# danielsuo/cuSIFT

Measured on AMD Instinct MI355X. Metric: Mpix/s pyramid + keypoints/s end-to-end, 1920x1080 batch, higher is better.
Workload: dtype f32

## Files before the change

### cusift_amd/csrc/detect_chunk.inc

```
  const int c0 = bx * kDetStrip - kDetHaloLanes * kBlurCols + lane * kBlurCols;
  const EdgeFix4 edge(c0, w);
  const __amdgpu_buffer_rsrc_t rin =
      __builtin_amdgcn_make_buffer_rsrc((void *)img, 0, (int)((unsigned int)h * (unsigned int)pitch * 4u), kBufFlags);
  const bool lane_valid = lane >= kDetHaloLanes && lane < 64 - kDetHaloLanes;

  auto load_raw = [&](int y) -> f4 {
    const int yc = clampi(__builtin_amdgcn_readfirstlane(y), 0, h - 1);
    return __builtin_bit_cast(f4, __builtin_amdgcn_raw_buffer_load_b128(rin, edge.voff, yc * pitch * 4, 0));
  };
  const bool edge_wave = bx == 0 || bx * kDetStrip - kDetHaloLanes * kBlurCols + 64 * kBlurCols > w;
  auto fix = [&](f4 v) -> f4 { return edge_wave ? edge(v) : v; };

  f4 win[9];
#pragma unroll
  for (int i = 0; i < 9; ++i) win[i] = fix(load_raw(ya - 1 - 4 + i));

  f4 DA[kNumDog], DB[kNumDog], DC[kNumDog];
#pragma unroll
  for (int p = 0; p < kNumDog; ++p) DA[p] = DB[p] = DC[p] = f4{0.f, 0.f, 0.f, 0.f};

  f2 hm1 = f2{0.f, 0.f}, h0 = hm1, hp1 = hm1;
  int voff_down = kOobOffset;
  if (kDown) {
    const bool odd0 = ((ya - 1) & 1) != 0;
    hm1 = down_hrow(odd0 ? win[4] : win[3], DT.k[0], DT.k[1], DT.k[2]);
    h0 = down_hrow(odd0 ? win[5] : win[4], DT.k[0], DT.k[1], DT.k[2]);
    hp1 = down_hrow(odd0 ? win[6] : win[5], DT.k[0], DT.k[1], DT.k[2]);
    voff_down = (lane_valid && c0 >= 0) ? (c0 >> 1) * 4 : kOobOffset;
  }

  f4 ahead = load_raw(ya - 1 + 5);
  auto row_step = [&](int yy, f4 (&D0)[kNumDog], f4 (&D1)[kNumDog], f4 (&D2)[kNumDog]) {
    const f4 nxt = ahead;
    ahead = load_raw(yy + 6);
    if (kDown) {
      const int yu = __builtin_amdgcn_readfirstlane(yy);
      if ((yu & 1) == 0) {
        const f2 hp2 = down_hrow(win[6], DT.k[0], DT.k[1], DT.k[2]), hp3 = down_hrow(win[7], DT.k[0], DT.k[1], DT.k[2]);
        const f2 o = down_vcol(hm1, h0, hp1, hp2, hp3, DT.k[0], DT.k[1], DT.k[2]);
        const int r = yu >> 1;
        if (yu >= own_lo && yu < own_hi && r < (h >> 1)) {
          const __amdgpu_buffer_rsrc_t ro = __builtin_amdgcn_make_buffer_rsrc(
              (void *)(down_img + (long)r * down_pitch), 0, (w >> 1) * 4, kBufFlags);
          __builtin_amdgcn_raw_buffer_store_b64(__builtin_bit_cast(u2, o), ro, voff_down, 0, 0);
        }
        hm1 = hp1;
        h0 = hp2;
        hp1 = hp3;
      }
    }
    blur_dog_row<kIdent0>(win, T, D2);

    if (yy >= ya + 1) {
      const int y = yy - 1;
      float vmax = 0.0f;
#pragma unroll
      for (int s = 0; s < kNumScales; ++s) {
        const f4 v = D1[s + 1];
        vmax = max3f(vmax, fabsf(v.x), fabsf(v.y));
        vmax = max3f(vmax, fabsf(v.z), fabsf(v.w));
      }
      const bool big = vmax > P.thr_pos && lane_valid && c0 < w;
      unsigned int cand = 0;
      if (__builtin_amdgcn_ballot_w64(big) != 0) {
        f4 hmn[kNumDog], hmx[kNumDog];
        f4 lmn[kNumScales], rmn[kNumScales], lmx[kNumScales], rmx[kNumScales];
#pragma unroll
        for (int p = 0; p < kNumDog; ++p) {
          f4 cmn, cmx, l_mn, r_mn, l_mx, r_mx;
#pragma unroll
          for (int j = 0; j < 4; ++j) {
            cmn[j] = min3f(D0[p][j], D1[p][j], D2[p][j]);
            cmx[j] = max3f(D0[p][j], D1[p][j], D2[p][j]);
          }
          l_mn = f4{from_prev_lane(cmn[3]), cmn[0], cmn[1], cmn[2]};
          r_mn = f4{cmn[1], cmn[2], cmn[3], from_next_lane(cmn[0])};
          l_mx = f4{from_prev_lane(cmx[3]), cmx[0], cmx[1], cmx[2]};
          r_mx = f4{cmx[1], cmx[2], cmx[3], from_next_lane(cmx[0])};
#pragma unroll
          for (int j = 0; j < 4; ++j) {
            hmn[p][j] = min3f(l_mn[j], cmn[j], r_mn[j]);
            hmx[p][j] = max3f(l_mx[j], cmx[j], r_mx[j]);
          }
          if (p >= 1 && p <= kNumScales) {
            lmn[p - 1] = l_mn;
            rmn[p - 1] = r_mn;
            lmx[p - 1] = l_mx;
            rmx[p - 1] = r_mx;
          }
        }
#pragma unroll
        for (int s = 0; s < kNumScales; ++s) {
          const int c = s + 1;
#pragma unroll
          for (int j = 0; j < 4; ++j) {
            const float v = D1[c][j];
            const float mn_a = min3f(lmn[s][j], rmn[s][j], D0[c][j]);
            const float mn_b = min3f(D2[c][j], hmn[c - 1][j], hmn[c + 1][j]);
            const float mx_a = max3f(lmx[s][j], rmx[s][j], D0[c][j]);
            const float mx_b = max3f(D2[c][j], hmx[c - 1][j], hmx[c + 1][j]);
            const bool hit = (v < min3f(mn_a, mn_b, P.thr_neg)) || (v > max3f(mx_a, mx_b, P.thr_pos));
            cand |= (hit ? 1u : 0u) << (4 * s + j);
          }
        }
      }
      if (!lane_valid) cand = 0;
#pragma unroll
      for (int j = 0; j < 4; ++j)
        if (c0 + j < 1 || c0 + j > w - 2) cand &= ~(0x11111u << j);
      if (__builtin_amdgcn_ballot_w64(cand != 0) != 0) {
#pragma unroll 1
        for (int s = 0; s < kNumScales; ++s) {
          const unsigned int m = (cand >> (4 * s)) & 0xfu;
          if (__builtin_amdgcn_ballot_w64(m != 0) == 0) continue;
          auto emit = [&](auto scale_c) {
            constexpr int k = decltype(scale_c)::value;
            auto column = [&](auto col_c) {
              constexpr int j = decltype(col_c)::value;
              const bool mine = (m >> j) & 1u;
              if (__builtin_amdgcn_ballot_w64(mine) == 0) return;
              auto at = [&](const f4 (&D)[kNumDog], int p, int dx) -> float {
                const int col = j + dx;
                if (col < 0) return from_prev_lane(D[p][3]);
                if (col > 3) return from_next_lane(D[p][0]);
                return D[p][col];
              };
              const float c00 = at(D0, k + 1, -1), c01 = at(D0, k + 1, 0), c02 = at(D0, k + 1, 1);
              const float c10 = at(D1, k + 1, -1), c11 = at(D1, k + 1, 0), c12 = at(D1, k + 1, 1);
              const float c20 = at(D2, k + 1, -1), c21 = at(D2, k + 1, 0), c22 = at(D2, k + 1, 1);
              const float l0 = at(D1, k, 0), l1 = at(D1, k, -1), l2 = at(D1, k, 1), l3 = at(D0, k, 0), l4 = at(D2, k, 0);
              const float h0 = at(D1, k + 2, 0), h1 = at(D1, k + 2, -1), h2 = at(D1, k + 2, 1), h3 = at(D0, k + 2, 0),
                          h4 = at(D2, k + 2, 0);
              float *e = cands.reserve(mine);
              if (mine) {
                e[0] = c00, e[1] = c01, e[2] = c02, e[3] = c10, e[4] = c11, e[5] = c12, e[6] = c20, e[7] = c21, e[8] = c22;
                e[9] = l0, e[10] = l1, e[11] = l2, e[12] = l3, e[13] = l4;
                e[14] = h0, e[15] = h1, e[16] = h2, e[17] = h3, e[18] = h4;
                e[19] = __builtin_bit_cast(float, c0 + j);
                e[20] = __builtin_bit_cast(float, ((y + rw.row0) << 3) | k);
              }
              if (cands.n >= 64) {
                cands.refine_batch<kRecBytes>(list, max_pts, counter, P, lane);
              }
            };
            column(std::integral_constant<int, 0>{});
            column(std::integral_constant<int, 1>{});
            column(std::integral_constant<int, 2>{});
            column(std::integral_constant<int, 3>{});
          };
          switch (s) {
            case 0: emit(std::integral_constant<int, 0>{}); break;
            case 1: emit(std::integral_constant<int, 1>{}); break;
            case 2: emit(std::integral_constant<int, 2>{}); break;
            case 3: emit(std::integral_constant<int, 3>{}); break;
            default: emit(std::integral_constant<int, 4>{}); break;
          }
        }
      }
    }
#pragma unroll
    for (int i = 0; i < 8; ++i) win[i] = win[i + 1];
    win[8] = fix(nxt);
  };

  for (int yy = ya - 1; yy <= yb; yy += 3) {
    row_step(yy, DA, DB, DC);
    if (yy + 1 > yb) break;
    row_step(yy + 1, DB, DC, DA);
    if (yy + 2 > yb) break;
    row_step(yy + 2, DC, DA, DB);
  }
  cands.refine_batch<kRecBytes>(list, max_pts, counter, P, lane);
```

### cusift_amd/csrc/sift_stencils.hip

```cpp
#include <type_traits>

#include "sift_device.h"

namespace cusift {

__global__ void __launch_bounds__(256) scale_down_kernel(float *__restrict__ dst, int dst_pitch, long dst_stride,
                                                        const float *__restrict__ src, int w, int h, int src_pitch,
                                                        long src_stride, int rows_per_wave, ScaleDownTaps T) {
  const int lane = threadIdx.x & 63;
  const int wv = __builtin_amdgcn_readfirstlane(threadIdx.x >> 6);
  const int ow = w >> 1, oh = h >> 1;
  const int c = blockIdx.x * 64 + lane;
  const int r0 = (blockIdx.y * kWavesPerBlock + wv) * rows_per_wave;
  if (r0 >= oh) return;
  const int r1 = min(r0 + rows_per_wave, oh);
  src += (long)blockIdx.z * src_stride;
  dst += (long)blockIdx.z * dst_stride;
  const int x0 = clampi(2 * c - 2, 0, w - 1), x1 = clampi(2 * c - 1, 0, w - 1), x2 = clampi(2 * c, 0, w - 1),
            x3 = clampi(2 * c + 1, 0, w - 1), x4 = clampi(2 * c + 2, 0, w - 1);
  const float k0 = T.k[0], k1 = T.k[1], k2 = T.k[2];
  auto hrow = [&](int y) -> float {
    const float *s = src + (long)clampi(y, 0, h - 1) * src_pitch;
    float v = k0 * (s[x0] + s[x4]);
    v = fmaf(k1, s[x1] + s[x3], v);
    v = fmaf(k2, s[x2], v);
    return v;
  };
  float bm1 = hrow(2 * r0 - 1), b0 = hrow(2 * r0), bp1 = hrow(2 * r0 + 1);
  for (int r = r0; r < r1; ++r) {
    const float bp2 = hrow(2 * r + 2), bp3 = hrow(2 * r + 3);
    float v = k2 * b0;
    v = fmaf(k0, bp3 + bp2, v);
    v = fmaf(k1, bm1 + bp1, v);
    if (c < ow) dst[(long)r * dst_pitch + c] = v;
    bm1 = bp1;
    b0 = bp2;
    bp1 = bp3;
  }
}

__global__ void __launch_bounds__(256) laplace_multi_kernel(const float *__restrict__ img, float *__restrict__ dog,
                                                           int w, int h, int pitch, long img_stride, long dog_stride,
                                                           int rows_per_wave, int vec_ok, LaplaceTaps T) {
  const int lane = threadIdx.x & 63;
  const int wv = __builtin_amdgcn_readfirstlane(threadIdx.x >> 6);
  const int y0 = (blockIdx.y * kWavesPerBlock + wv) * rows_per_wave;
  if (y0 >= h) return;
  const int y1 = min(y0 + rows_per_wave, h);
  img += (long)blockIdx.z * img_stride;
  dog += (long)blockIdx.z * dog_stride;

  const int c0 = blockIdx.x * kBlurStrip - kBlurHaloLanes * kBlurCols + lane * kBlurCols;
  const bool interior = vec_ok && c0 >= 0 && c0 + 3 < w;
  const int cc0 = clampi(c0, 0, w - 1), cc1 = clampi(c0 + 1, 0, w - 1), cc2 = clampi(c0 + 2, 0, w - 1),
            cc3 = clampi(c0 + 3, 0, w - 1);

  float win[9][4];
  auto load_row = [&](int y, float (&o)[4]) {
    const float *r = img + (long)clampi(y, 0, h - 1) * pitch;
    if (interior) {
      const float4 v = *reinterpret_cast<const float4 *>(r + c0);
      o[0] = v.x; o[1] = v.y; o[2] = v.z; o[3] = v.w;
    } else {
      o[0] = r[cc0]; o[1] = r[cc1]; o[2] = r[cc2]; o[3] = r[cc3];
    }
  };
#pragma unroll
  for (int i = 0; i < 8; ++i) load_row(y0 - 4 + i, win[i]);

  const bool writer = lane >= kBlurHaloLanes && lane < 64 - kBlurHaloLanes && c0 < w;
  const bool vec_store = vec_ok && (c0 + 3 < w);
  const long plane = (long)h * pitch;

  for (int y = y0; y < y1; ++y) {
    load_row(y + 4, win[8]);
    float ctr[4], p1[4], p2[4], p3[4], p4[4];
#pragma unroll
    for (int j = 0; j < 4; ++j) {
      ctr[j] = win[4][j];
      p1[j] = win[3][j] + win[5][j];
      p2[j] = win[2][j] + win[6][j];
      p3[j] = win[1][j] + win[7][j];
      p4[j] = win[0][j] + win[8][j];
    }
    float prevL[4];
    float *out = dog + (long)y * pitch + c0;
#pragma unroll
    for (int s = 0; s < kNumLevels; ++s) {
      const float k0 = T.k[s][0], k1 = T.k[s][1], k2 = T.k[s][2], k3 = T.k[s][3], k4 = T.k[s][4];
      float e[12];
#pragma unroll
      for (int j = 0; j < 4; ++j) {
        float v = k4 * ctr[j];
        v = fmaf(k3, p1[j], v);
        v = fmaf(k2, p2[j], v);
        v = fmaf(k1, p3[j], v);
        v = fmaf(k0, p4[j], v);
        e[4 + j] = v;
      }
#pragma unroll
      for (int j = 0; j < 4; ++j) {
        e[j] = from_prev_lane(e[4 + j]);
        e[8 + j] = from_next_lane(e[4 + j]);
      }
      float L[4];
#pragma unroll
      for (int j = 0; j < 4; ++j) {
        const int m = 4 + j;
        float v = k4 * e[m];
        v = fmaf(k3, e[m - 1] + e[m + 1], v);
        v = fmaf(k2, e[m - 2] + e[m + 2], v);
        v = fmaf(k1, e[m - 3] + e[m + 3], v);
        v = fmaf(k0, e[m - 4] + e[m + 4], v);
        L[j] = v;
      }
      if (s > 0 && writer) {
        float *o = out + (long)(s - 1) * plane;
        if (vec_store) {
          *reinterpret_cast<float4 *>(o) =
              make_float4(prevL[0] - L[0], prevL[1] - L[1], prevL[2] - L[2], prevL[3] - L[3]);
        } else {
#pragma unroll
          for (int j = 0; j < 4; ++j)
            if (c0 + j < w) o[j] = prevL[j] - L[j];
        }
      }
#pragma unroll
      for (int j = 0; j < 4; ++j) prevL[j] = L[j];
    }
#pragma unroll
    for (int i = 0; i < 8; ++i)
#pragma unroll
      for (int j = 0; j < 4; ++j) win[i][j] = win[i + 1][j];
  }
}

__device__ __forceinline__ f2 splat(float v) { return f2{v, v}; }
__device__ __forceinline__ f2 pk_fma(f2 a, f2 b, f2 c) { return __builtin_elementwise_fma(a, b, c); }
__device__ __forceinline__ f2 dpp_prev2(f2 v) { return f2{from_prev_lane(v.x), from_prev_lane(v.y)}; }
__device__ __forceinline__ f2 dpp_next2(f2 v) { return f2{from_next_lane(v.x), from_next_lane(v.y)}; }

template <int kStoreAux>
__global__ void __launch_bounds__(256) laplace_multi_fast_kernel(const float *__restrict__ img,
                                                                float *__restrict__ dog, int w, int h, int pitch,
                                                                long img_stride, long dog_stride, int rows_per_wave,
                                                                LaplaceTapsPk T) {
  const int lane = threadIdx.x & 63;
  const int wv = __builtin_amdgcn_readfirstlane(threadIdx.x >> 6);
  int bx = blockIdx.x, by = blockIdx.y, bz = blockIdx.z;
  xcd_remap(bx, by, bz);
  const int y0 = (by * (int)(blockDim.x >> 6) + wv) * rows_per_wave;
  if (y0 >= h) return;
  const int y1 = min(y0 + rows_per_wave, h);
  img += (long)bz * img_stride;
  dog += (long)bz * dog_stride;

  const int c0 = bx * kBlurStrip - kBlurHaloLanes * kBlurCols + lane * kBlurCols;
  const EdgeFix4 edge(c0, w);
  const __amdgpu_buffer_rsrc_t rin =
      __builtin_amdgcn_make_buffer_rsrc((void *)img, 0, (int)((unsigned int)h * (unsigned int)pitch * 4u), kBufFlags);
  const int voff_out = (lane >= kBlurHaloLanes && lane < 64 - kBlurHaloLanes) ? c0 * 4 : kOobOffset;
  const long plane = (long)h * pitch;

  auto load_row = [&](int y) -> f4 {
    const int yc = clampi(y, 0, h - 1);
    const u4 raw = __builtin_amdgcn_raw_buffer_load_b128(rin, edge.voff, yc * pitch * 4, 0);
    return edge(__builtin_bit_cast(f4, raw));
  };

  f4 win[9];
#pragma unroll
  for (int i = 0; i < 9; ++i) win[i] = load_row(y0 - 4 + i);

  for (int y = y0; y < y1; ++y) {
    const f4 nxt = load_row(y + 5);
    const f4 ctr = win[4];
    const f4 p1 = win[3] + win[5];
    const f4 p2 = win[2] + win[6];
    const f4 p3 = win[1] + win[7];
    const f4 p4 = win[0] + win[8];
    float *row = dog + (long)y * pitch;
    float prev_hi[4];
#pragma unroll
    for (int q = 0; q < kNumLevels / 2; ++q) {
      const f2 k0 = T.k[q][0], k1 = T.k[q][1], k2 = T.k[q][2], k3 = T.k[q][3], k4 = T.k[q][4];
      f2 e[12];
#pragma unroll
      for (int j = 0; j < 4; ++j) {
        f2 v = k4 * splat(ctr[j]);
        v = pk_fma(k3, splat(p1[j]), v);
        v = pk_fma(k2, splat(p2[j]), v);
        v = pk_fma(k1, splat(p3[j]), v);
        v = pk_fma(k0, splat(p4[j]), v);
        e[4 + j] = v;
      }
#pragma unroll
      for (int j = 0; j < 4; ++j) {
        e[j] = dpp_prev2(e[4 + j]);
        e[8 + j] = dpp_next2(e[4 + j]);
      }
      f2 L[4];
#pragma unroll
      for (int j = 0; j < 4; ++j) {
        const int m = 4 + j;
        f2 v = k4 * e[m];
        v = pk_fma(k3, e[m - 1] + e[m + 1], v);
        v = pk_fma(k2, e[m - 2] + e[m + 2], v);
        v = pk_fma(k1, e[m - 3] + e[m + 3], v);
        v = pk_fma(k0, e[m - 4] + e[m + 4], v);
        L[j] = v;
      }
      if (q > 0) {
        const f4 d = f4{prev_hi[0] - L[0].x, prev_hi[1] - L[1].x, prev_hi[2] - L[2].x, prev_hi[3] - L[3].x};
        const __amdgpu_buffer_rsrc_t ro =
            __builtin_amdgcn_make_buffer_rsrc((void *)(row + (long)(2 * q - 1) * plane), 0, w * 4, kBufFlags);
        __builtin_amdgcn_raw_buffer_store_b128(__builtin_bit_cast(u4, d), ro, voff_out, 0, kStoreAux);
      }
      {
        const f4 d = f4{L[0].x - L[0].y, L[1].x - L[1].y, L[2].x - L[2].y, L[3].x - L[3].y};
        if (2 * q < kNumDog) {
          const __amdgpu_buffer_rsrc_t ro =
              __builtin_amdgcn_make_buffer_rsrc((void *)(row + (long)(2 * q) * plane), 0, w * 4, kBufFlags);
          __builtin_amdgcn_raw_buffer_store_b128(__builtin_bit_cast(u4, d), ro, voff_out, 0, kStoreAux);
        }
      }
#pragma unroll
      for (int j = 0; j < 4; ++j) prev_hi[j] = L[j].y;
    }
#pragma unroll
    for (int i = 0; i < 8; ++i) win[i] = win[i + 1];
    win[8] = nxt;
  }
}
template __global__ void laplace_multi_fast_kernel<2>(const float *, float *, int, int, int, long, long, int, LaplaceTapsPk);

constexpr int kDownStrip = 62 * 2;

__device__ __forceinline__ f2 down_hrow(const f4 v, float k0, float k1, float k2) {
  const float m2 = from_prev_lane(v.z), m1 = from_prev_lane(v.w), p4 = from_next_lane(v.x);
  float a = k0 * (m2 + v.z);
  a = fmaf(k1, m1 + v.y, a);
  a = fmaf(k2, v.x, a);
  float b = k0 * (v.x + p4);
  b = fmaf(k1, v.y + v.w, b);
  b = fmaf(k2, v.z, b);
  return f2{a, b};
}
__device__ __forceinline__ f2 down_vcol(f2 bm1, f2 b0, f2 bp1, f2 bp2, f2 bp3, float k0, float k1, float k2) {
  f2 v;
#pragma unroll
  for (int j = 0; j < 2; ++j) {
    float t = k2 * b0[j];
    t = fmaf(k0, bp3[j] + bp2[j], t);
    t = fmaf(k1, bm1[j] + bp1[j], t);
    v[j] = t;
  }
  return v;
}

__global__ void __launch_bounds__(256) scale_down_fast_kernel(float *__restrict__ dst, int dst_pitch, long dst_stride,
                                                             const float *__restrict__ src, int w, int h,
                                                             int src_pitch, long src_stride, int rows_per_wave,
                                                             ScaleDownTaps T, RowWindow src_rw, int dst_row0,
                                                             int r_begin, int r_end) {
  const int lane = threadIdx.x & 63;
  const int wv = __builtin_amdgcn_readfirstlane(threadIdx.x >> 6);
  int bx = blockIdx.x, by = blockIdx.y, bz = blockIdx.z;
  xcd_remap(bx, by, bz);
  const int ow = w >> 1;
  const int strip = bx * kWavesPerBlock + wv;
  const int r0 = r_begin + by * rows_per_wave;
  if (strip * kDownStrip >= ow || r0 >= r_end) return;
  const int r1 = min(r0 + rows_per_wave, r_end);
  src += (long)bz * src_stride;
  dst += (long)bz * dst_stride;

  const int cs = strip * (2 * kDownStrip) - 4 + lane * 4;
  const EdgeFix4 edge(cs, w);
  const __amdgpu_buffer_rsrc_t rin = __builtin_amdgcn_make_buffer_rsrc(
      (void *)src, 0, (int)((unsigned int)h * (unsigned int)src_pitch * 4u), kBufFlags);
  const int o0 = cs >> 1;
  const int voff_out = (lane >= 1 && lane <= 62 && cs >= 0) ? o0 * 4 : kOobOffset;
  const float k0 = T.k[0], k1 = T.k[1], k2 = T.k[2];

  auto load_row = [&](int y) -> f4 {
    const u4 raw = __builtin_amdgcn_raw_buffer_load_b128(rin, edge.voff, local_row(y, h, src_rw) * src_pitch * 4, 0);
    return edge(__builtin_bit_cast(f4, raw));
  };
  auto hrow = [&](const f4 v) -> f2 { return down_hrow(v, k0, k1, k2); };

  f2 bm1 = hrow(load_row(2 * r0 - 1)), b0 = hrow(load_row(2 * r0)), bp1 = hrow(load_row(2 * r0 + 1));
  f4 n2 = load_row(2 * r0 + 2), n3 = load_row(2 * r0 + 3);
  for (int r = r0; r < r1; ++r) {
    const f4 s2 = n2, s3 = n3;
    n2 = load_row(2 * r + 4);
    n3 = load_row(2 * r + 5);
    const f2 bp2 = hrow(s2), bp3 = hrow(s3);
    const f2 v = down_vcol(bm1, b0, bp1, bp2, bp3, k0, k1, k2);
    const __amdgpu_buffer_rsrc_t ro =
        __builtin_amdgcn_make_buffer_rsrc((void *)(dst + (long)(r - dst_row0) * dst_pitch), 0, ow * 4, kBufFlags);
    __builtin_amdgcn_raw_buffer_store_b64(__builtin_bit_cast(u2, v), ro, voff_out, 0, 0);
    bm1 = bp1;
    b0 = bp2;
    bp1 = bp3;
  }
}

struct RefinedPoint {
  float x, y, scale, sharpness, edgeness;
};

__device__ __forceinline__ bool refine_from_values(const float (&c)[9], const float (&lo)[5], const float (&hi)[5], int x,
                                                   int y, int s, const FindParams &P, RefinedPoint &r) {
  const float val = c[4];
  const float dxx = 2.0f * val - c[3] - c[5];
  const float dyy = 2.0f * val - c[1] - c[7];
  const float dxy = 0.25f * (c[8] + c[0] - c[2] - c[6]);
  const float tra = dxx + dyy;
  const float det = dxx * dyy - dxy * dxy;
  if (!(tra * tra < P.edge_limit * det)) return false;
  const float edge = (tra * tra) / det;
  const float dx = 0.5f * (c[5] - c[3]);
  const float dy = 0.5f * (c[7] - c[1]);
  const float ds = 0.5f * (lo[0] - hi[0]);
  const float dss = 2.0f * val - hi[0] - lo[0];
  const float dxs = 0.25f * (hi[2] + lo[1] - lo[2] - hi[1]);
  const float dys = 0.25f * (hi[4] + lo[3] - hi[3] - lo[4]);
  const float idxx = dyy * dss - dys * dys;
  const float idxy = dys * dxs - dxy * dss;
  const float idxs = dxy * dys - dyy * dxs;
  const float idet = 1.0f / (idxx * dxx + idxy * dxy + idxs * dxs);
  const float idyy = dxx * dss - dxs * dxs;
  const float idys = dxy * dxs - dxx * dys;
  const float idss = dxx * dyy - dxy * dxy;
  float pdx = idet * (idxx * dx + idxy * dy + idxs * ds);
  float pdy = idet * (idxy * dx + idyy * dy + idys * ds);
  float pds = idet * (idxs * dx + idys * dy + idss * ds);
  if (pdx < -0.5f || pdx > 0.5f || pdy < -0.5f || pdy > 0.5f || pds < -0.5f || pds > 0.5f) {
    pdx = dx / dxx;
    pdy = dy / dyy;
    pds = ds / dss;
  }
  const float dval = 0.5f * (dx * pdx + dy * pdy + ds * pds);
  r.x = (float)x + pdx;
  r.y = (float)y + pdy;
  r.scale = P.scales[s] * sm_exp2f(pds * P.factor);
  r.sharpness = val + dval;
  r.edgeness = edge;
  return true;
}

__device__ __forceinline__ void load_candidate(const float *__restrict__ dog, long plane, int pitch, int x, int y, int s,
                                               float (&c)[9], float (&lo)[5], float (&hi)[5]) {
  const float *d1 = dog + (long)(s + 1) * plane + (long)y * pitch + x;
  const float *d0 = d1 - plane;
  const float *d2 = d1 + plane;
#pragma unroll
  for (int r = 0; r < 3; ++r)
#pragma unroll
    for (int k = 0; k < 3; ++k) c[3 * r + k] = d1[(r - 1) * pitch + (k - 1)];
  lo[0] = d0[0], lo[1] = d0[-1], lo[2] = d0[1], lo[3] = d0[-pitch], lo[4] = d0[pitch];
  hi[0] = d2[0], hi[1] = d2[-1], hi[2] = d2[1], hi[3] = d2[-pitch], hi[4] = d2[pitch];
}

__device__ __forceinline__ bool refine_from_planes(const float *__restrict__ dog, long plane, int pitch, int x, int y,
                                                   int s, const FindParams &P, RefinedPoint &r) {
  float c[9], lo[5], hi[5];
  load_candidate(dog, plane, pitch, x, y, s, c, lo, hi);
  return refine_from_values(c, lo, hi, x, y, s, P, r);
}

constexpr int kPosCap = 128;
struct PosList {
  unsigned int *buf;
  int n;
  __device__ __forceinline__ void push(bool mine, int x, int y, int s) {
    const unsigned long long m = __builtin_amdgcn_ballot_w64(mine);
    if (m == 0) return;
    const int rank = __builtin_amdgcn_mbcnt_hi((unsigned int)(m >> 32), __builtin_amdgcn_mbcnt_lo((unsigned int)m, 0u));
    if (mine) {
      buf[2 * (n + rank)] = (unsigned int)x | ((unsigned int)s << 28);
      buf[2 * (n + rank) + 1] = (unsigned int)y;
    }
    n += __builtin_popcountll(m);
  }
  __device__ __forceinline__ void refine_batch(const float *__restrict__ dog, long plane, int pitch,
                                               cusift_point *__restrict__ pts, int max_pts, unsigned int *counter,
                                               const FindParams &P, int lane) {
    const int cnt = n < 64 ? n : 64;
    if (cnt == 0) return;
    n -= cnt;
    asm volatile("s_waitcnt lgkmcnt(0)" ::: "memory");
    RefinedPoint r;
    bool accept = false;
    if (lane < cnt) {
      const unsigned int xs = buf[2 * (n + lane)], y = buf[2 * (n + lane) + 1];
      accept = refine_from_planes(dog, plane, pitch, (int)(xs & 0x0fffffffu), (int)y, (int)(xs >> 28), P, r);
    }
    const unsigned long long m = __builtin_amdgcn_ballot_w64(accept);
    if (m == 0) return;
    const int rank = __builtin_amdgcn_mbcnt_hi((unsigned int)(m >> 32), __builtin_amdgcn_mbcnt_lo((unsigned int)m, 0u));
    unsigned int base = 0;
    if (lane == 0) base = atomicAdd(counter, (unsigned int)__builtin_popcountll(m));
    base = __builtin_amdgcn_readfirstlane(base);
    const unsigned int idx = base + (unsigned int)rank;
    if (accept && idx < (unsigned int)max_pts) {
      cusift_point *pt = pts + idx;
      pt->coords2D[0] = r.x;
      pt->coords2D[1] = r.y;
      pt->scale = r.scale;
      pt->sharpness = r.sharpness;
      pt->edgeness = r.edgeness;
      pt->subsampling = P.subsampling;
    }
  }
};

__device__ __forceinline__ void refine_and_append(const float *__restrict__ dog, long plane, int pitch, int x, int y,
                                                   int s, const FindParams &P, cusift_point *__restrict__ pts,
                                                   int max_pts, unsigned int *counter) {
  RefinedPoint r;
  if (!refine_from_planes(dog, plane, pitch, x, y, s, P, r)) return;
  const unsigned int idx = atomicAdd(counter, 1u);
  if (idx >= (unsigned int)max_pts) return;
  cusift_point *pt = pts + idx;
  pt->coords2D[0] = r.x;
  pt->coords2D[1] = r.y;
  pt->scale = r.scale;
  pt->sharpness = r.sharpness;
  pt->edgeness = r.edgeness;
  pt->subsampling = P.subsampling;
}

__global__ void __launch_bounds__(256) find_points_kernel(const float *__restrict__ dog, int w, int h, int pitch,
                                                         long dog_stride, cusift_point *__restrict__ points,
                                                         int max_pts, unsigned int *__restrict__ counters,
                                                         int rows_per_wave, int vec_ok, FindParams P) {
  const int lane = threadIdx.x & 63;
  const int wv = __builtin_amdgcn_readfirstlane(threadIdx.x >> 6);
  const int y0 = (blockIdx.y * kWavesPerBlock + wv) * rows_per_wave;
  if (y0 >= h) return;
  const int y1 = min(y0 + rows_per_wave, h);
  dog += (long)blockIdx.z * dog_stride;
  points += (long)blockIdx.z * max_pts;
  unsigned int *counter = counters + blockIdx.z;

  const int c0 = blockIdx.x * kFindStrip - kFindCols + lane * kFindCols;
  const bool interior = vec_ok && c0 >= 0 && c0 + 1 < w;
  const int cc0 = clampi(c0, 0, w - 1), cc1 = clampi(c0 + 1, 0, w - 1);
  const long plane = (long)h * pitch;

  float d[kNumDog][3][2];
  auto load_rows = [&](int y, int slot) {
    const float *r = dog + (long)clampi(y, 0, h - 1) * pitch;
#pragma unroll
    for (int p = 0; p < kNumDog; ++p) {
      if (interior) {
        const float2 v = *reinterpret_cast<const float2 *>(r + (long)p * plane + c0);
        d[p][slot][0] = v.x;
        d[p][slot][1] = v.y;
      } else {
        d[p][slot][0] = r[(long)p * plane + cc0];
        d[p][slot][1] = r[(long)p * plane + cc1];
      }
    }
  };
  load_rows(y0 - 1, 0);
  load_rows(y0, 1);
  const bool lane_valid = lane >= 1 && lane <= 62;

  for (int y = y0; y < y1; ++y) {
    load_rows(y + 1, 2);
    float cmin[kNumDog][2], cmax[kNumDog][2], nmin[kNumDog][2][2], nmax[kNumDog][2][2];
#pragma unroll
    for (int p = 0; p < kNumDog; ++p) {
#pragma unroll
      for (int j = 0; j < 2; ++j) {
        cmin[p][j] = fminf(fminf(d[p][0][j], d[p][1][j]), d[p][2][j]);
        cmax[p][j] = fmaxf(fmaxf(d[p][0][j], d[p][1][j]), d[p][2][j]);
      }
      nmin[p][0][0] = from_prev_lane(cmin[p][1]);
      nmin[p][0][1] = cmin[p][1];
      nmin[p][1][0] = cmin[p][0];
      nmin[p][1][1] = from_next_lane(cmin[p][0]);
      nmax[p][0][0] = from_prev_lane(cmax[p][1]);
      nmax[p][0][1] = cmax[p][1];
      nmax[p][1][0] = cmax[p][0];
      nmax[p][1][1] = from_next_lane(cmax[p][0]);
    }
    unsigned int cand = 0;
#pragma unroll
    for (int s = 0; s < kNumScales; ++s) {
      const int c = s + 1;
#pragma unroll
      for (int j = 0; j < 2; ++j) {
        const float v = d[c][1][j];
        float mn = fminf(fminf(nmin[c - 1][j][0], cmin[c - 1][j]), nmin[c - 1][j][1]);
        mn = fminf(mn, fminf(fminf(nmin[c + 1][j][0], cmin[c + 1][j]), nmin[c + 1][j][1]));
        mn = fminf(mn, fminf(fminf(nmin[c][j][0], nmin[c][j][1]), fminf(d[c][0][j], d[c][2][j])));
        float mx = fmaxf(fmaxf(nmax[c - 1][j][0], cmax[c - 1][j]), nmax[c - 1][j][1]);
        mx = fmaxf(mx, fmaxf(fmaxf(nmax[c + 1][j][0], cmax[c + 1][j]), nmax[c + 1][j][1]));
        mx = fmaxf(mx, fmaxf(fmaxf(nmax[c][j][0], nmax[c][j][1]), fmaxf(d[c][0][j], d[c][2][j])));
        const bool hit = (v < P.thr_neg && v < mn) || (v > P.thr_pos && v > mx);
        cand |= (hit ? 1u : 0u) << (2 * s + j);
      }
    }
    if (!lane_valid) cand = 0;
    if (cand) {
      for (int b = 0; b < 2 * kNumScales; ++b) {
        if (cand & (1u << b)) {
          const int x = c0 + (b & 1), s = b >> 1;
          if (x >= 1 && x <= w - 2 && y >= 1 && y <= h - 2)
            refine_and_append(dog, plane, pitch, x, y, s, P, points, max_pts, counter);
        }
      }
    }
#pragma unroll
    for (int p = 0; p < kNumDog; ++p)
#pragma unroll
      for (int j = 0; j < 2; ++j) {
        d[p][0][j] = d[p][1][j];
        d[p][1][j] = d[p][2][j];
      }
  }
}

__device__ __forceinline__ float min3f(float a, float b, float c) { return fminf(fminf(a, b), c); }
__device__ __forceinline__ float max3f(float a, float b, float c) { return fmaxf(fmaxf(a, b), c); }

__global__ void __launch_bounds__(256) find_points_fast_kernel(const float *__restrict__ dog, int w, int h, int pitch,
                                                              long dog_stride, cusift_point *__restrict__ points,
                                                              int max_pts, unsigned int *__restrict__ counters,
                                                              int rows_per_wave, FindParams P) {
  const int lane = threadIdx.x & 63;
  const int wv = __builtin_amdgcn_readfirstlane(threadIdx.x >> 6);
  int bx = blockIdx.x, by = blockIdx.y, bz = blockIdx.z;
  xcd_remap(bx, by, bz);
  const int strip = bx * kWavesPerBlock + wv;
  const int y0 = by * rows_per_wave;
  if (strip * kFindStrip >= w || y0 >= h) return;
  const int y1 = min(y0 + rows_per_wave, h);
  dog += (long)bz * dog_stride;
  points += (long)bz * max_pts;
  unsigned int *counter = counters + bz;

  const int c0 = strip * kFindStrip - kFindCols + lane * kFindCols;
  const EdgeFix2 edge(c0, w);
  const long plane = (long)h * pitch;
  const int plane_bytes = (int)((unsigned int)h * (unsigned int)pitch * 4u);
  const __amdgpu_buffer_rsrc_t rin =
      __builtin_amdgcn_make_buffer_rsrc((void *)dog, 0, (int)((unsigned int)plane_bytes * (unsigned int)kNumDog), kBufFlags);

  auto load_row = [&](int y, f2 (&o)[kNumDog]) {
    const int row_off = clampi(y, 0, h - 1) * pitch * 4;
#pragma unroll
    for (int p = 0; p < kNumDog; ++p) {
      const u2 raw = __builtin_amdgcn_raw_buffer_load_b64(rin, edge.voff, p * plane_bytes + row_off, 0);
      o[p] = edge(__builtin_bit_cast(f2, raw));
    }
  };

  __shared__ unsigned int s_cands[kWavesPerBlock][2 * kPosCap];
  PosList cands{s_cands[wv], 0};
  f2 r0[kNumDog], r1[kNumDog], r2[kNumDog], nxt[kNumDog];
  load_row(y0 - 1, r0);
  load_row(y0, r1);
  load_row(y0 + 1, r2);
  const bool lane_valid = lane >= 1 && lane <= 62;

  for (int y = y0; y < y1; ++y) {
    load_row(y + 2, nxt);
    float cmn[kNumDog][2], cmx[kNumDog][2], hmn[kNumDog][2], hmx[kNumDog][2], lmn[kNumDog], rmn[kNumDog],
        lmx[kNumDog], rmx[kNumDog];
#pragma unroll
    for (int p = 0; p < kNumDog; ++p) {
#pragma unroll
      for (int j = 0; j < 2; ++j) {
        cmn[p][j] = min3f(r0[p][j], r1[p][j], r2[p][j]);
        cmx[p][j] = max3f(r0[p][j], r1[p][j], r2[p][j]);
      }
      lmn[p] = from_prev_lane(cmn[p][1]);
      rmn[p] = from_next_lane(cmn[p][0]);
      lmx[p] = from_prev_lane(cmx[p][1]);
      rmx[p] = from_next_lane(cmx[p][0]);
      hmn[p][0] = min3f(lmn[p], cmn[p][0], cmn[p][1]);
      hmn[p][1] = min3f(cmn[p][0], cmn[p][1], rmn[p]);
      hmx[p][0] = max3f(lmx[p], cmx[p][0], cmx[p][1]);
      hmx[p][1] = max3f(cmx[p][0], cmx[p][1], rmx[p]);
    }
    unsigned int cand = 0;
#pragma unroll
    for (int s = 0; s < kNumScales; ++s) {
      const int c = s + 1;
#pragma unroll
      for (int j = 0; j < 2; ++j) {
        const float v = r1[c][j];
        const float nl_mn = j == 0 ? lmn[c] : cmn[c][0], nr_mn = j == 0 ? cmn[c][1] : rmn[c];
        const float nl_mx = j == 0 ? lmx[c] : cmx[c][0], nr_mx = j == 0 ? cmx[c][1] : rmx[c];
        const float mn_a = min3f(nl_mn, nr_mn, r0[c][j]);
        const float mn_b = min3f(r2[c][j], hmn[c - 1][j], hmn[c + 1][j]);
        const float mx_a = max3f(nl_mx, nr_mx, r0[c][j]);
        const float mx_b = max3f(r2[c][j], hmx[c - 1][j], hmx[c + 1][j]);
        const bool hit = (v < min3f(mn_a, mn_b, P.thr_neg)) || (v > max3f(mx_a, mx_b, P.thr_pos));
        cand |= (hit ? 1u : 0u) << (2 * s + j);
      }
    }
    if (!lane_valid) cand = 0;
    if (__builtin_amdgcn_ballot_w64(cand != 0) != 0) {
      for (int b = 0; b < 2 * kNumScales; ++b) {
        const int x = c0 + (b & 1), s = b >> 1;
        const bool mine = (cand & (1u << b)) && x >= 1 && x <= w - 2 && y >= 1 && y <= h - 2;
        cands.push(mine, x, y, s);
        if (cands.n >= 64) cands.refine_batch(dog, plane, pitch, points, max_pts, counter, P, lane);
      }
    }
#pragma unroll
    for (int p = 0; p < kNumDog; ++p) {
      r0[p] = r1[p];
      r1[p] = r2[p];
      r2[p] = nxt[p];
    }
  }
  cands.refine_batch(dog, plane, pitch, points, max_pts, counter, P, lane);
}

constexpr int kDetHaloLanes = 2;
constexpr int kDetStrip = (64 - 2 * kDetHaloLanes) * kBlurCols;
constexpr int kCandWords = 21;
constexpr int kCandCap = 128;
static_assert(kCandCap * kCandWords == kDetectWaveLdsFloats, "host and kernel agree on the LDS size");

template <bool kIdent0>
__device__ __forceinline__ void blur_dog_row(const f4 (&win)[9], const LaplaceTapsPk &T, f4 (&D)[kNumDog]) {
  const f4 ctr = win[4];
  const f4 p1 = win[3] + win[5];
  const f4 p2 = win[2] + win[6];
  const f4 p3 = win[1] + win[7];
  const f4 p4 = win[0] + win[8];
  float prev_hi[4];
  if (kIdent0) {
    D[0] = f4{0.f, 0.f, 0.f, 0.f};
#pragma unroll
    for (int j = 0; j < 4; ++j) prev_hi[j] = ctr[j];
  }
#pragma unroll
  for (int q = kIdent0 ? 1 : 0; q < kNumLevels / 2; ++q) {
    const f2 k0 = T.k[q][0], k1 = T.k[q][1], k2 = T.k[q][2], k3 = T.k[q][3], k4 = T.k[q][4];
    f2 e[12];
#pragma unroll
    for (int j = 0; j < 4; ++j) {
      f2 v = k4 * splat(ctr[j]);
      v = pk_fma(k3, splat(p1[j]), v);
      v = pk_fma(k2, splat(p2[j]), v);
      v = pk_fma(k1, splat(p3[j]), v);
      v = pk_fma(k0, splat(p4[j]), v);
      e[4 + j] = v;
    }
#pragma unroll
    for (int j = 0; j < 4; ++j) {
      e[j] = dpp_prev2(e[4 + j]);
      e[8 + j] = dpp_next2(e[4 + j]);
    }
    f2 L[4];
#pragma unroll
    for (int j = 0; j < 4; ++j) {
      const int m = 4 + j;
      f2 v = k4 * e[m];
      v = pk_fma(k3, e[m - 1] + e[m + 1], v);
      v = pk_fma(k2, e[m - 2] + e[m + 2], v);
      v = pk_fma(k1, e[m - 3] + e[m + 3], v);
      v = pk_fma(k0, e[m - 4] + e[m + 4], v);
      L[j] = v;
    }
    if (q > 0) D[2 * q - 1] = f4{prev_hi[0] - L[0].x, prev_hi[1] - L[1].x, prev_hi[2] - L[2].x, prev_hi[3] - L[3].x};
    if (2 * q < kNumDog) D[2 * q] = f4{L[0].x - L[0].y, L[1].x - L[1].y, L[2].x - L[2].y, L[3].x - L[3].y};
#pragma unroll
    for (int j = 0; j < 4; ++j) prev_hi[j] = L[j].y;
  }
}

struct CandList {
  float *buf;
  int n;
  __device__ __forceinline__ float *reserve(bool mine) {
    const unsigned long long m = __builtin_amdgcn_ballot_w64(mine);
    const int rank = __builtin_amdgcn_mbcnt_hi((unsigned int)(m >> 32), __builtin_amdgcn_mbcnt_lo((unsigned int)m, 0u));
    float *e = mine ? buf + (n + rank) * kCandWords : nullptr;
    n += __builtin_popcountll(m);
    return e;
  }
  template <int kRecBytes>
  __device__ __forceinline__ void refine_batch(char *__restrict__ pts, int max_pts, unsigned int *counter,
                                               const FindParams &P, int lane) {
    const int cnt = n < 64 ? n : 64;
    if (cnt == 0) return;
    n -= cnt;
    asm volatile("s_waitcnt lgkmcnt(0)" ::: "memory");
    RefinedPoint r;
    bool accept = false;
    if (lane < cnt) {
      const float *e = buf + (n + lane) * kCandWords;
      float c[9], lo[5], hi[5];
#pragma unroll
      for (int k = 0; k < 9; ++k) c[k] = e[k];
#pragma unroll
      for (int k = 0; k < 5; ++k) lo[k] = e[9 + k], hi[k] = e[14 + k];
      const int x = __builtin_bit_cast(int, e[19]);
      const int ys = __builtin_bit_cast(int, e[20]);
      accept = refine_from_values(c, lo, hi, x, ys >> 3, ys & 7, P, r);
    }
    const unsigned long long m = __builtin_amdgcn_ballot_w64(accept);
    if (m == 0) return;
    const int rank = __builtin_amdgcn_mbcnt_hi((unsigned int)(m >> 32), __builtin_amdgcn_mbcnt_lo((unsigned int)m, 0u));
    unsigned int base = 0;
    if (lane == 0) base = atomicAdd(counter, (unsigned int)__builtin_popcountll(m));
    base = __builtin_amdgcn_readfirstlane(base);
    const unsigned int idx = base + (unsigned int)rank;
    if (accept && idx < (unsigned int)max_pts) {
      cusift_point *pt = reinterpret_cast<cusift_point *>(pts + (size_t)idx * kRecBytes);
      pt->coords2D[0] = r.x;
      pt->coords2D[1] = r.y;
      pt->scale = r.scale;
      pt->sharpness = r.sharpness;
      pt->edgeness = r.edgeness;
      pt->subsampling = P.subsampling;
    }
  }
};

template <bool kIdent0, int kRecBytes, bool kDown>
__global__ void __launch_bounds__(256) __attribute__((amdgpu_waves_per_eu(2))) detect_fused_kernel(const float *__restrict__ img, int w, int h, int pitch,
                                                          long img_stride, cusift_point *__restrict__ points,
                                                          int max_pts, unsigned int *__restrict__ counters,
                                                          int rows_per_wave, LaplaceTapsPk T, FindParams P,
                                                          RowWindow rw, int cy_begin, int cy_end, DownOut down) {
  extern __shared__ float s_cands[];
  const int lane = threadIdx.x & 63;
  const int wv = __builtin_amdgcn_readfirstlane(threadIdx.x >> 6);
  int bx = blockIdx.x, by = blockIdx.y, bz = blockIdx.z;
  xcd_remap(bx, by, bz);
  const int gy0 = cy_begin + (by * (int)(blockDim.x >> 6) + wv) * rows_per_wave;
  const int ya = max(max(gy0, 1), cy_begin) - rw.row0;
  const int yb = min(min(gy0 + rows_per_wave, rw.hg - 1), cy_end) - rw.row0;
  if (ya >= yb) return;
  img += (long)bz * img_stride;
  char *const list = reinterpret_cast<char *>(points) + (size_t)bz * max_pts * kRecBytes;
  unsigned int *counter = counters + bz;
  CandList cands{s_cands + wv * kDetectWaveLdsFloats, 0};
  const int own_lo = gy0, own_hi = gy0 + rows_per_wave;
  float *const down_img = kDown ? down.dst + (long)bz * down.stride : nullptr;
  const int down_pitch = down.pitch;
  const ScaleDownTaps DT = down.T;

#include "detect_chunk.inc"
}


struct PyrRange {
  int x0, x1, y0, y1;
  __device__ __forceinline__ int w() const { return x1 - x0; }
  __device__ __forceinline__ int h() const { return y1 - y0; }
};

__global__ void __launch_bounds__(256) pyramid_small_kernel(PyramidLevels P, ScaleDownTaps T, unsigned int *zero,
                                                            int n_zero) {
  extern __shared__ float s_pyr[];
  const int tid = threadIdx.x;
  if (blockIdx.x == 0 && blockIdx.y == 0 && blockIdx.z == 0)
    for (int i = tid; i < n_zero; i += 256) zero[i] = 0u;
  const long img = blockIdx.z;
  PyrRange own[kMaxPyramidLevels + 2], need[kMaxPyramidLevels + 2];
#pragma unroll
  for (int k = kMaxPyramidLevels; k >= 1; --k) {
    if (k > P.n) continue;
    if (k == P.n) {
      own[k].x0 = blockIdx.x * P.tile;
      own[k].y0 = blockIdx.y * P.tile;
      own[k].x1 = min(own[k].x0 + P.tile, P.w[k]);
      own[k].y1 = min(own[k].y0 + P.tile, P.h[k]);
      need[k] = own[k];
    } else {
      own[k].x0 = 2 * own[k + 1].x0;
      own[k].y0 = 2 * own[k + 1].y0;
      own[k].x1 = own[k + 1].x1 == P.w[k + 1] ? P.w[k] : 2 * own[k + 1].x1;
      own[k].y1 = own[k + 1].y1 == P.h[k + 1] ? P.h[k] : 2 * own[k + 1].y1;
      need[k].x0 = min(own[k].x0, max(2 * need[k + 1].x0 - 2, 0));
      need[k].x1 = max(own[k].x1, min(2 * (need[k + 1].x1 - 1) + 2, P.w[k] - 1) + 1);
      need[k].y0 = min(own[k].y0, max(2 * need[k + 1].y0 - 1, 0));
      need[k].y1 = max(own[k].y1, min(2 * (need[k + 1].y1 - 1) + 3, P.h[k] - 1) + 1);
    }
  }
  need[0] = own[0] = PyrRange{0, 0, 0, 0};
  const float k0 = T.k[0], k1 = T.k[1], k2 = T.k[2];
  float *lvl[kMaxPyramidLevels + 1];
  float *cursor = s_pyr;
  lvl[0] = nullptr;
#pragma unroll
  for (int k = 1; k <= kMaxPyramidLevels; ++k) {
    lvl[k] = cursor;
    if (k <= P.n) cursor += need[k].w() * need[k].h();
  }
  float *const H = cursor;

#pragma unroll
  for (int k = 1; k <= kMaxPyramidLevels; ++k) {
    if (k > P.n) break;
    const int sw = P.w[k - 1], sh = P.h[k - 1];
    const PyrRange N = need[k];
    const int nw = N.w();
    const int ry0 = max(2 * N.y0 - 1, 0), ry1 = min(2 * (N.y1 - 1) + 3, sh - 1);
    const int hrows = ry1 - ry0 + 1;
    const float *src0 = P.base[0] + img * P.stride[0];
    const PyrRange S = need[k - 1];
    const int spw = k >= 2 ? S.w() : 0;
    for (int e = tid; e < hrows * nw; e += 256) {
      const int yy = e / nw, cc = e - yy * nw;
      const int y = ry0 + yy, c = N.x0 + cc;
      const int xa = max(2 * c - 2, 0), xb = max(2 * c - 1, 0), xc = 2 * c, xd = min(2 * c + 1, sw - 1), xe = min(2 * c + 2, sw - 1);
      float a0, a1, a2, a3, a4;
      if (k == 1) {
        const float *r = src0 + (long)y * P.pitch[0];
        a0 = r[xa], a1 = r[xb], a2 = r[min(xc, sw - 1)], a3 = r[xd], a4 = r[xe];
      } else {
        const float *r = lvl[k - 1] + (y - S.y0) * spw - S.x0;
        a0 = r[xa], a1 = r[xb], a2 = r[min(xc, sw - 1)], a3 = r[xd], a4 = r[xe];
      }
      float v = k0 * (a0 + a4);
      v = fmaf(k1, a1 + a3, v);
      v = fmaf(k2, a2, v);
      H[e] = v;
    }
    __syncthreads();
    float *dst = P.base[k] + img * P.stride[k];
    const PyrRange O = own[k];
    for (int e = tid; e < N.h() * nw; e += 256) {
      const int rr = e / nw, cc = e - rr * nw;
      const int r = N.y0 + rr, c = N.x0 + cc;
      const float *h = H + cc;
      auto row = [&](int y) { return h[(min(max(y, 0), sh - 1) - ry0) * nw]; };
      float v = k2 * row(2 * r);
      v = fmaf(k0, row(2 * r + 3) + row(2 * r + 2), v);
      v = fmaf(k1, row(2 * r - 1) + row(2 * r + 1), v);
      lvl[k][e] = v;
      if (r >= O.y0 && r < O.y1 && c >= O.x0 && c < O.x1) dst[(long)r * P.pitch[k] + c] = v;
    }
    __syncthreads();
  }
}

template <int kRecBytes>
__global__ void __launch_bounds__(64) __attribute__((amdgpu_waves_per_eu(2))) detect_multi_kernel(DetectTable tab, int max_pts,
                                                                                          unsigned int *queue) {
  extern __shared__ float s_cands[];
  const int lane = threadIdx.x;
  const int b = blockIdx.x;
  if (b == 0 && queue)
    for (int i = lane; i < kQueueShards * 32; i += 64) queue[i] = 0u;
  int oi = 0;
  while (oi + 1 < tab.n && b >= tab.o[oi + 1].first_block) ++oi;
  const DetectOctave &O = tab.o[oi];
  const int local = b - O.first_block;
  const int bx = local % O.strips;
  const int by = (local / O.strips) % O.chunks;
  const int bz = local / (O.strips * O.chunks);
  const int w = O.w, h = O.h, pitch = O.pitch;
  const RowWindow rw{O.row0, O.hg};
  const int gy0 = O.cy_begin + by * O.rows_per_wave;
  const int ya = max(max(gy0, 1), O.cy_begin) - rw.row0;
  const int yb = min(min(gy0 + O.rows_per_wave, rw.hg - 1), O.cy_end) - rw.row0;
  if (ya >= yb) return;
  const float *img = O.img + (long)bz * O.img_stride;
  char *const list = O.lists + (size_t)bz * max_pts * kRecBytes;
  unsigned int *counter = O.counters + bz;
  CandList cands{s_cands, 0};
  const LaplaceTapsPk &T = O.T;
  const FindParams &P = O.P;
  constexpr bool kDown = false;
  constexpr int own_lo = 0, own_hi = 0, down_pitch = 0;
  float *const down_img = nullptr;
  const ScaleDownTaps DT{};
  if (O.ident) {
    constexpr bool kIdent0 = true;
#include "detect_chunk.inc"
  } else {
    constexpr bool kIdent0 = false;
#include "detect_chunk.inc"
  }
}

template __global__ void detect_multi_kernel<kStagedRecBytes>(DetectTable, int, unsigned int *);

#define CUSIFT_DETECT_INSTANCE(IDENT, REC, DOWN)                                                                     \
  template __global__ void detect_fused_kernel<IDENT, REC, DOWN>(const float *, int, int, int, long, cusift_point *,  \
                                                                 int, unsigned int *, int, LaplaceTapsPk, FindParams, \
                                                                 RowWindow, int, int, DownOut);
CUSIFT_DETECT_INSTANCE(false, (int)sizeof(cusift_point), false)
CUSIFT_DETECT_INSTANCE(true, (int)sizeof(cusift_point), false)
CUSIFT_DETECT_INSTANCE(false, kStagedRecBytes, false)
CUSIFT_DETECT_INSTANCE(true, kStagedRecBytes, false)
CUSIFT_DETECT_INSTANCE(false, kStagedRecBytes, true)
CUSIFT_DETECT_INSTANCE(true, kStagedRecBytes, true)
#undef CUSIFT_DETECT_INSTANCE

}
```

Before: 143,200.

## Use separable cube min/max with equality test and exact recheck for DoG extrema

Replaces the per-scale 26-neighbour extremum test with a separable 3x3x3 min/max: it builds horizontal 3-wide min/max per DoG plane, folds in scale neighbours and thresholds (nudged one ulp so that equality still means strictly past the threshold), then flags candidates where the centre equals the cube min or max. Because the equality test also accepts ties, each flagged column is re-checked exactly against its 26 neighbours before it is emitted. The plane-0 work is skipped when it is an identity plane. This cuts ALU and cross-lane shuffle work in the hot per-row path, at the cost of extra work in the rarer emit path.

```diff
diff --git a/cusift_amd/csrc/detect_chunk.inc b/cusift_amd/csrc/detect_chunk.inc
--- a/cusift_amd/csrc/detect_chunk.inc
+++ b/cusift_amd/csrc/detect_chunk.inc
@@ -64,42 +64,41 @@
       unsigned int cand = 0;
       if (__builtin_amdgcn_ballot_w64(big) != 0) {
         f4 hmn[kNumDog], hmx[kNumDog];
-        f4 lmn[kNumScales], rmn[kNumScales], lmx[kNumScales], rmx[kNumScales];
 #pragma unroll
         for (int p = 0; p < kNumDog; ++p) {
-          f4 cmn, cmx, l_mn, r_mn, l_mx, r_mx;
+          if (kIdent0 && p == 0) {
+            hmn[0] = hmx[0] = f4{0.f, 0.f, 0.f, 0.f};
+            continue;
+          }
+          f4 cmn, cmx;
 #pragma unroll
           for (int j = 0; j < 4; ++j) {
             cmn[j] = min3f(D0[p][j], D1[p][j], D2[p][j]);
             cmx[j] = max3f(D0[p][j], D1[p][j], D2[p][j]);
           }
-          l_mn = f4{from_prev_lane(cmn[3]), cmn[0], cmn[1], cmn[2]};
-          r_mn = f4{cmn[1], cmn[2], cmn[3], from_next_lane(cmn[0])};
-          l_mx = f4{from_prev_lane(cmx[3]), cmx[0], cmx[1], cmx[2]};
-          r_mx = f4{cmx[1], cmx[2], cmx[3], from_next_lane(cmx[0])};
+          const float l_mn = from_prev_lane(cmn[3]), r_mn = from_next_lane(cmn[0]);
+          const float l_mx = from_prev_lane(cmx[3]), r_mx = from_next_lane(cmx[0]);
+          hmn[p] = f4{min3f(l_mn, cmn[0], cmn[1]), min3f(cmn[0], cmn[1], cmn[2]), min3f(cmn[1], cmn[2], cmn[3]),
+                      min3f(cmn[2], cmn[3], r_mn)};
+          hmx[p] = f4{max3f(l_mx, cmx[0], cmx[1]), max3f(cmx[0], cmx[1], cmx[2]), max3f(cmx[1], cmx[2], cmx[3]),
+                      max3f(cmx[2], cmx[3], r_mx)};
+        }
+        static_assert(kNumDog == 7 && kNumScales == 5, "cube windows below");
+        const float lo = float_below(P.thr_neg), hi = float_above(P.thr_pos);
 #pragma unroll
-          for (int j = 0; j < 4; ++j) {
-            hmn[p][j] = min3f(l_mn[j], cmn[j], r_mn[j]);
-            hmx[p][j] = max3f(l_mx[j], cmx[j], r_mx[j]);
-          }
-          if (p >= 1 && p <= kNumScales) {
-            lmn[p - 1] = l_mn;
-            rmn[p - 1] = r_mn;
-            lmx[p - 1] = l_mx;
-            rmx[p - 1] = r_mx;
-          }
-        }
+        for (int j = 0; j < 4; ++j) {
+          const float n2 = fminf(hmn[2][j], lo), n5 = fminf(hmn[5][j], lo);
+          const float x2 = fmaxf(hmx[2][j], hi), x5 = fmaxf(hmx[5][j], hi);
+          const float cube_mn[kNumScales] = {min3f(hmn[0][j], hmn[1][j], n2), min3f(hmn[1][j], n2, hmn[3][j]),
+                                             min3f(n2, hmn[3][j], hmn[4][j]), min3f(hmn[3][j], hmn[4][j], n5),
+                                             min3f(hmn[4][j], n5, hmn[6][j])};
+          const float cube_mx[kNumScales] = {max3f(hmx[0][j], hmx[1][j], x2), max3f(hmx[1][j], x2, hmx[3][j]),
+                                             max3f(x2, hmx[3][j], hmx[4][j]), max3f(hmx[3][j], hmx[4][j], x5),
+                                             max3f(hmx[4][j], x5, hmx[6][j])};
 #pragma unroll
-        for (int s = 0; s < kNumScales; ++s) {
-          const int c = s + 1;
-#pragma unroll
-          for (int j = 0; j < 4; ++j) {
-            const float v = D1[c][j];
-            const float mn_a = min3f(lmn[s][j], rmn[s][j], D0[c][j]);
-            const float mn_b = min3f(D2[c][j], hmn[c - 1][j], hmn[c + 1][j]);
-            const float mx_a = max3f(lmx[s][j], rmx[s][j], D0[c][j]);
-            const float mx_b = max3f(D2[c][j], hmx[c - 1][j], hmx[c + 1][j]);
-            const bool hit = (v < min3f(mn_a, mn_b, P.thr_neg)) || (v > max3f(mx_a, mx_b, P.thr_pos));
+          for (int s = 0; s < kNumScales; ++s) {
+            const float v = D1[s + 1][j];
+            const bool hit = v == cube_mn[s] || v == cube_mx[s];
             cand |= (hit ? 1u : 0u) << (4 * s + j);
           }
         }
@@ -117,8 +116,7 @@
             constexpr int k = decltype(scale_c)::value;
             auto column = [&](auto col_c) {
               constexpr int j = decltype(col_c)::value;
-              const bool mine = (m >> j) & 1u;
-              if (__builtin_amdgcn_ballot_w64(mine) == 0) return;
+              if (__builtin_amdgcn_ballot_w64((m >> j) & 1u) == 0) return;
               auto at = [&](const f4 (&D)[kNumDog], int p, int dx) -> float {
                 const int col = j + dx;
                 if (col < 0) return from_prev_lane(D[p][3]);
@@ -131,6 +129,14 @@
               const float l0 = at(D1, k, 0), l1 = at(D1, k, -1), l2 = at(D1, k, 1), l3 = at(D0, k, 0), l4 = at(D2, k, 0);
               const float h0 = at(D1, k + 2, 0), h1 = at(D1, k + 2, -1), h2 = at(D1, k + 2, 1), h3 = at(D0, k + 2, 0),
                           h4 = at(D2, k + 2, 0);
+              const float nb[26] = {c00, c01, c02, c10, c12, c20, c21, c22,
+                                    l0, l1, l2, l3, l4, at(D0, k, -1), at(D0, k, 1), at(D2, k, -1), at(D2, k, 1),
+                                    h0, h1, h2, h3, h4, at(D0, k + 2, -1), at(D0, k + 2, 1), at(D2, k + 2, -1),
+                                    at(D2, k + 2, 1)};
+              float nmn = INFINITY, nmx = -INFINITY;
+#pragma unroll
+              for (int i = 0; i < 26; ++i) nmn = fminf(nmn, nb[i]), nmx = fmaxf(nmx, nb[i]);
+              const bool mine = ((m >> j) & 1u) && ((c11 < P.thr_neg && c11 < nmn) || (c11 > P.thr_pos && c11 > nmx));
               float *e = cands.reserve(mine);
               if (mine) {
                 e[0] = c00, e[1] = c01, e[2] = c02, e[3] = c10, e[4] = c11, e[5] = c12, e[6] = c20, e[7] = c21, e[8] = c22;
diff --git a/cusift_amd/csrc/sift_stencils.hip b/cusift_amd/csrc/sift_stencils.hip
--- a/cusift_amd/csrc/sift_stencils.hip
+++ b/cusift_amd/csrc/sift_stencils.hip
@@ -527,6 +527,12 @@
 
 __device__ __forceinline__ float min3f(float a, float b, float c) { return fminf(fminf(a, b), c); }
 __device__ __forceinline__ float max3f(float a, float b, float c) { return fmaxf(fmaxf(a, b), c); }
+__device__ __forceinline__ float float_above(float x) {
+  int b = __builtin_bit_cast(int, x);
+  if (b == (int)0x80000000) b = 0;
+  return __builtin_bit_cast(float, b >= 0 ? b + 1 : b - 1);
+}
+__device__ __forceinline__ float float_below(float x) { return -float_above(-x); }
 
 __global__ void __launch_bounds__(256) find_points_fast_kernel(const float *__restrict__ dog, int w, int h, int pitch,
                                                               long dog_stride, cusift_point *__restrict__ points,
```

New measurement: 123,300 (median of 2 runs). 13.9% lower.
